# planck-epoch/unet-image-segmentation

Measured on AMD Instinct MI355X. Metric: images/sec (train step, 256x256x3), higher is better.
Workload: dtype f32; 1 GPU; configs[1]: 256x256x3 binary U-Net train step (fwd + dice_loss + bwd + AdamW + MeanIoU(2) update, dropout 0.2); network=U_NET separable-conv, filters 64-128-256-512, bneck 1024, global_batch=16, per_gpu_batch=16, seq_len=65536, parallelism=dp1, batchnorm=per-replica

## Files before the change

unet-image-segmentation_amd/csrc/gemm.hip:

```cpp
#include <cstdlib>
#include "dispatch.h"
#include "view.h"

namespace unet {

int colsum(const float* x, int64_t rows, int cols, float* out, void* ws, size_t ws_bytes, hipStream_t st);
size_t bn_partials_bytes(int64_t m, int c);
size_t colsum_workspace(int64_t rows, int cols);

namespace {

constexpr int BK = 16;

enum { A_PLAIN = 0, A_BNRELU = 1, A_UNSHUFFLE = 2, A_BNBWD = 3 };
enum { E_STORE = 0, E_STATS = 1, E_SHUFFLE = 2, E_BNPART = 3 };

struct RowsArgs {
    DView a;
    int64_t M;
    int K;
    int uH, uW, uf;
    const float* B;
    int64_t sbk, sbn;
    int N;
    float* C;
    int64_t ldc;
    const float* bias;
    float2* stats;
    int sH, sW, sf;
    const float* z;
    const float* coef;
    float* side;
    const float *bsc, *bsh, *bmu, *brs;
    float* bnpart;
    float ep_rate, ep_inv_keep;
    uint64_t ep_seed;
    int ko;
    const unsigned short* Bx;
};
#ifdef UNET_LAB_BUILD
#define ROWS_KO(g, bit) (((g).ko & (bit)) != 0)
#else
#define ROWS_KO(g, bit) false
#endif

__device__ __forceinline__ int acc_row(int r, int hi) { return (r & 3) + 8 * (r >> 2) + 4 * hi; }

__device__ __forceinline__ void xcd_group_order(int groups, int sibs, int& grp, int& sib) {
    grp = blockIdx.x;
    sib = blockIdx.y;
    if (sibs > 1 && (groups & 7) == 0) {
        const int L = blockIdx.x + blockIdx.y * groups, u = L >> 3;
        grp = (u / sibs) * 8 + (L & 7);
        sib = u % sibs;
    }
// ... 183 lines not shown
            if (hi == 0) red[wm * BN + col] = q;
        }
        __syncthreads();
        if (wm == 0 && hi == 0) {
#pragma unroll
            for (int tn = 0; tn < TN; ++tn) {
                const int col = wn * (BN / 2) + tn * 32 + lo;
                const int n = n0 + col;
                if (n < g.N) g.stats[(int64_t)blockIdx.x * g.N + n] = make_float2(mean[tn], red[col] + red[BN + col]);
            }
        }
    }
    if constexpr (EPI == E_SHUFFLE) {
        const int64_t hw = (int64_t)g.sH * g.sW;
#pragma unroll
        for (int tn = 0; tn < TN; ++tn) {
            const int n = n0 + wn * (BN / 2) + tn * 32 + lo;
            if (n >= g.N) continue;
            const int ab = n / g.sf;
            const int co = n - ab * g.sf;
            const int a = ab >> 1, b = ab & 1;
            const float bias = g.bias ? g.bias[co] : 0.f;
#pragma unroll
            for (int tm = 0; tm < TM; ++tm)
#pragma unroll
                for (int r = 0; r < 16; ++r) {
                    const int rr = wm * (BM / 2) + tm * 32 + acc_row(r, hi);
                    if (rr >= M_rem) continue;
                    const int64_t m = m0 + rr;
                    const int img = (int)(m / hw);
                    const int rem = (int)(m - img * hw);
                    const int i = rem / g.sW, j = rem - (rem / g.sW) * g.sW;
                    const int64_t o = ((int64_t)(img * 2 * g.sH + 2 * i + a) * (2 * g.sW) + 2 * j + b) * g.sf + co;
                    g.C[o] = acc[tm][tn][r] + bias;
                }
        }
    }
}

enum { W_PLAIN = 0, W_BNRELU = 1, W_UNSHUFFLE = 2, W_BNBWD = 3 };

struct WgradArgs {
    DView a;
    int P;
    int uH, uW, uf;
    DView b;
    int Q;
    int64_t M, mslice;
    float* slab;
    const float* bz;
    const float* bcoef;
    float* colpart;
    bool x6;
};

template <int BP, int BQ, int AMODE, bool ADROP, int BMODE, bool BDROP>
__global__ __launch_bounds__(256) void gemm_wgrad_kernel(WgradArgs g) {
    constexpr int LDA = BP + 4, LDB = BQ + 4;
    constexpr int TM = BP / 64, TN = BQ / 64;
    constexpr int AR = BP / 16, BR = BQ / 16;
    constexpr int AS = 256 / BP, BS = 256 / BQ;
    __shared__ float As[2][BK][LDA];
    __shared__ float Bs[2][BK][LDB];

    const int tid = threadIdx.x, lane = tid & 63, wave = tid >> 6;
    const int wp = wave >> 1, wq = wave & 1;
    const int lo = lane & 31, hi = lane >> 5;
    const int ntp = (g.P + BP - 1) / BP;
    const int p0 = (blockIdx.x % ntp) * BP;
    const int q0 = (blockIdx.x / ntp) * BQ;
    const int64_t mb = (int64_t)blockIdx.y * g.mslice;
    const int64_t me = mb + g.mslice < g.M ? mb + g.mslice : g.M;

    const int ap = tid % BP, amm = tid / BP;
    const int p = p0 + ap;
    const bool pv = p < g.P;
    float asc = 1.f, ash = 0.f;
    int poff = p;
    if constexpr (AMODE == W_BNRELU) {
        if (pv) {
            asc = g.a.sc0[p];
            ash = g.a.sh0[p];
        }
    }
    if constexpr (AMODE == W_UNSHUFFLE) {
        const int ab = p / g.uf;
        const int co = p - ab * g.uf;
        poff = (ab >> 1) * (2 * g.uW * g.uf) + (ab & 1) * g.uf + co;
    }
    const int bq = tid % BQ, bmm = tid / BQ;
    const int q = q0 + bq;
    const bool qv = q < g.Q;
    float bsc = 1.f, bsh = 0.f;
    if constexpr (BMODE == W_BNRELU) {
        if (qv) {
            bsc = g.b.sc0[q];
            bsh = g.b.sh0[q];
        }
    }

    float ra[AR], rb[BR];
    auto load_stage = [&](int64_t k0) {
#pragma unroll
        for (int r = 0; r < AR; ++r) {
            const int64_t m = k0 + amm + AS * r;
            float v = 0.f;
            if (pv && m < me) {
// ... 14 lines not shown
#pragma unroll
        for (int r = 0; r < BR; ++r) {
            const int64_t m = k0 + bmm + BS * r;
            float v = 0.f;
            if (qv && m < me) {
                v = g.b.src0[m * g.b.c0 + q];
                if constexpr (BMODE == W_BNRELU) v = bnrelu(v, bsc, bsh);
                if constexpr (BDROP) v *= drop_mult(g.b.seed, (uint64_t)m * g.b.C + q, g.b.rate, g.b.inv_keep);
            }
            rb[r] = v;
        }
    };
    auto store_stage = [&](int buf) {
#pragma unroll
        for (int r = 0; r < AR; ++r) As[buf][amm + AS * r][ap] = ra[r];
#pragma unroll
        for (int r = 0; r < BR; ++r) Bs[buf][bmm + BS * r][bq] = rb[r];
    };

    floatx16 acc[TM][TN];
#pragma unroll
    for (int tm = 0; tm < TM; ++tm)
#pragma unroll
        for (int tn = 0; tn < TN; ++tn)
#pragma unroll
            for (int r = 0; r < 16; ++r) acc[tm][tn][r] = 0.f;

    const int nk = (int)((me - mb + BK - 1) / BK);
    if (nk > 0) {
        load_stage(mb);
        store_stage(0);
    }
    __syncthreads();
    for (int kt = 0; kt < nk; ++kt) {
        const int buf = kt & 1;
        if (kt + 1 < nk) load_stage(mb + (int64_t)(kt + 1) * BK);
#pragma unroll
        for (int kk = 0; kk < BK / 2; ++kk) {
            float av[TM], bv[TN];
#pragma unroll
            for (int tm = 0; tm < TM; ++tm) av[tm] = As[buf][2 * kk + hi][wp * (BP / 2) + tm * 32 + lo];
#pragma unroll
            for (int tn = 0; tn < TN; ++tn) bv[tn] = Bs[buf][2 * kk + hi][wq * (BQ / 2) + tn * 32 + lo];
#pragma unroll
            for (int tm = 0; tm < TM; ++tm)
#pragma unroll
                for (int tn = 0; tn < TN; ++tn)
                    acc[tm][tn] = __builtin_amdgcn_mfma_f32_32x32x2f32(av[tm], bv[tn], acc[tm][tn], 0, 0, 0);
        }
        if (kt + 1 < nk) store_stage(buf ^ 1);
        __syncthreads();
    }
    float* slab = g.slab + (int64_t)blockIdx.y * g.P * g.Q;
#pragma unroll
    for (int tm = 0; tm < TM; ++tm)
#pragma unroll
        for (int tn = 0; tn < TN; ++tn) {
            const int qq = q0 + wq * (BQ / 2) + tn * 32 + lo;
            if (qq >= g.Q) continue;
#pragma unroll
            for (int r = 0; r < 16; ++r) {
                const int pp = p0 + wp * (BP / 2) + tm * 32 + acc_row(r, hi);
                if (pp < g.P) slab[(int64_t)pp * g.Q + qq] = acc[tm][tn][r];
            }
        }
}

#ifdef UNET_LAB_BUILD
__device__ __forceinline__ void lab_stagger(int ko) {
    const int n = (ko >> 8) & 255;
    if (n == 0) return;
    const unsigned lin = blockIdx.x + blockIdx.y * gridDim.x, tot = gridDim.x * gridDim.y;
    const bool late = (ko & 0x10000) ? (lin & 1) : (lin >= tot / 2);
    if (late)
        for (int i = 0; i < n; ++i) __builtin_amdgcn_s_sleep(32);
}
#define ROWS_STAGGER(g) lab_stagger((g).ko)
__device__ unsigned long long lab_rows_stamps[65536 * 4];
#define ROWS_STAMP(g, i)                                                                       \
    do {                                                                                       \
        if (((g).ko & 0x20000) && threadIdx.x == 0) {                                          \
            const unsigned lin_ = blockIdx.x + blockIdx.y * gridDim.x;                         \
            if (lin_ < 65536) lab_rows_stamps[4 * lin_ + (i)] =                               \
                ((i) == 0 || (i) == 3) ? __builtin_amdgcn_s_memrealtime() : __builtin_amdgcn_s_memtime(); \
        }                                                                                      \
    } while (0)
#else
#define ROWS_STAGGER(g) ((void)0)
#define ROWS_STAMP(g, i) ((void)0)
#endif

template <int BM, int BN, int BK, int AMODE, bool DROP, int EPI, bool BKC, bool X6 = false>
__global__ __launch_bounds__(256, X6 ? 2 : 1) void gemm_rows_vec(RowsArgs g) {
    main_stream_prio();
    ROWS_STAGGER(g);
    ROWS_STAMP(g, 0);
    constexpr int LR = BK + 4;
    constexpr int LB = BN + 4;
    constexpr int XR = BK + 8;
    constexpr int KQ = BK / 4;
    constexpr int NQ = BN / 4;
    constexpr int AQ = BM * KQ / 256;
    constexpr int BQ = BN * KQ / 256;
    constexpr int TM = BM / 64, TN = BN / 64;
    constexpr int BSZ = BKC ? BN * LR : BK * LB;
    constexpr int F32_BYTES = 4 * 2 * (BM * LR + BSZ);
    constexpr int X6_KMAX = 512;
    constexpr bool XCOEF = X6 && AMODE == A_BNBWD;
    constexpr int X6_BYTES = 2 * 3 * (BM + BN) * XR + (XCOEF ? 4 * 5 * X6_KMAX : 0);
    static_assert(!X6 || BK == 32, "X6 rows GEMM: 32-deep stages");
    __shared__ __attribute__((aligned(16))) char smem[X6 ? X6_BYTES : F32_BYTES];
    float* xcoef = reinterpret_cast<float*>(smem + 2 * 3 * (BM + BN) * XR);
    float (*As)[BM * LR] = reinterpret_cast<float (*)[BM * LR]>(smem);
    float (*Bs)[BSZ] = reinterpret_cast<float (*)[BSZ]>(smem + 4 * 2 * BM * LR);
    unsigned short* Ax = reinterpret_cast<unsigned short*>(smem);
    unsigned short* Bx = Ax + 3 * BM * XR;
    constexpr int XCH = BK / 8, XQ = 3 * BN * XCH / 256;
    static_assert(!X6 || (3 * BN * XCH) % 256 == 0, "X6: whole B chunks per thread");
// ... 348 lines not shown
                    }
                }
            }
            s1 += __shfl_xor(s1, 32, 64);
            s2 += __shfl_xor(s2, 32, 64);
            if (hi == 0) red[wm * BN + col] = make_float2(s1, s2);
        }
        __syncthreads();
        if (wm == 0 && hi == 0) {
            float* out = g.bnpart + (int64_t)mt * 2 * g.N;
#pragma unroll
            for (int tn = 0; tn < TN; ++tn) {
                const int col = wn * (BN / 2) + tn * 32 + lo;
                const int n = n0 + col;
                const float2 a = red[col], b = red[BN + col];
                if (n < g.N) {
                    out[n] = a.x + b.x;
                    out[g.N + n] = a.y + b.y;
                }
            }
        }
    }
    if constexpr (EPI == E_SHUFFLE) {
        int* orow = reinterpret_cast<int*>(&As[0][0]);
        if (tid < BM) {
            const int m = m0 + tid;
            const int ur = m / g.sW;
            orow[tid] = tid < M_rem ? (4 * ur * g.sW + 2 * (m - ur * g.sW)) * g.sf : -1;
        }
        __syncthreads();
        int obase[TM][16];
#pragma unroll
        for (int tm = 0; tm < TM; ++tm)
#pragma unroll
            for (int r = 0; r < 16; ++r) obase[tm][r] = orow[wm * (BM / 2) + tm * 32 + acc_row(r, hi)];
#pragma unroll
        for (int tn = 0; tn < TN; ++tn) {
            const int n = n0 + wn * (BN / 2) + tn * 32 + lo;
            if (n >= g.N) continue;
            const int ab = n / g.sf;
            const int co = n - ab * g.sf;
            const int toff = (ab >> 1) * (2 * g.sW * g.sf) + (ab & 1) * g.sf + co;
            const float bias = g.bias ? g.bias[co] : 0.f;
#pragma unroll
            for (int tm = 0; tm < TM; ++tm)
#pragma unroll
                for (int r = 0; r < 16; ++r)
                    if (obase[tm][r] >= 0) g.C[(int64_t)obase[tm][r] + toff] = acc[tm][tn][r] + bias;
        }
    }
    ROWS_STAMP(g, 3);
}

template <int BP, int BQ, int AMODE, bool ADROP, int BMODE, bool BDROP, bool X6 = false>
__global__ __launch_bounds__(256, X6 ? 2 : 1) void gemm_wgrad_vec(WgradArgs g) {
    static_assert(!X6 || (BP == 128 && BQ == 128), "X6 wgrad: 128 x 128 tiles");
    constexpr int KB = X6 ? 32 : BK;
    constexpr int LDA = BP + 4, LDB = BQ + 4;
    constexpr int TM = BP / 64, TN = BQ / 64;
    constexpr int PQ = BP / 4, QQ = BQ / 4;
    constexpr int AR = X6 ? 8 : BK * PQ / 256, BR = X6 ? 8 : BK * QQ / 256;
    constexpr int AS = X6 ? 1 : 256 / PQ, BS = X6 ? 1 : 256 / QQ;
    constexpr int XW = KB + 8;
    constexpr int F32_BYTES = 4 * 2 * BK * (LDA + LDB);
    constexpr int X6_BYTES = 2 * 3 * (BP + BQ) * XW;
    __shared__ __attribute__((aligned(16))) char smem[X6 ? X6_BYTES : F32_BYTES];
    float (*As)[BK * LDA] = reinterpret_cast<float (*)[BK * LDA]>(smem);
    float (*Bs)[BK * LDB] = reinterpret_cast<float (*)[BK * LDB]>(smem + 4 * 2 * BK * LDA);
    unsigned short* Ax = reinterpret_cast<unsigned short*>(smem);
    unsigned short* Bx = Ax + 3 * BP * XW;

    const int tid = threadIdx.x, lane = tid & 63, wave = tid >> 6;
    const int wp = wave >> 1, wq = wave & 1;
    const int lo = lane & 31, hi = lane >> 5;
    const int ntp = (g.P + BP - 1) / BP;
    int tile, slice;
    xcd_group_order_sx(gridDim.x, gridDim.y, tile, slice);
    const int p0 = (tile % ntp) * BP;
    const int q0 = (tile / ntp) * BQ;
    const int mb = (int)(slice * g.mslice);
    const int me = (int)((mb + g.mslice) < g.M ? (mb + g.mslice) : g.M);
    const bool roleA = !X6 || tid < 128, roleB = !X6 || tid >= 128;
    const int unit = tid & 127;

    const int apq = X6 ? unit >> 2 : tid % PQ, amm = X6 ? 8 * (unit & 3) : tid / PQ;
    const int p = p0 + 4 * apq;
    const bool pv = p < g.P;
    float4 asc = f4(1.f), ash = f4(0.f);
    int poff = p;
    if constexpr (AMODE == W_BNRELU) {
        if (pv) {
            asc = ld4(g.a.sc0 + p);
            ash = ld4(g.a.sh0 + p);
        }
    }
    if constexpr (AMODE == W_UNSHUFFLE) {
        const int ab = p / g.uf;
        const int co = p - ab * g.uf;
        poff = (ab >> 1) * (2 * g.uW * g.uf) + (ab & 1) * g.uf + co;
    }
    const int bqq = X6 ? unit >> 2 : tid % QQ, bmm = X6 ? 8 * (unit & 3) : tid / QQ;
    const int q = q0 + 4 * bqq;
    const bool qv = q < g.Q;
    float4 bsc = f4(1.f), bsh = f4(0.f), bmu = f4(0.f), bp_ = f4(0.f), bq_ = f4(0.f);
    if constexpr (BMODE == W_BNRELU || BMODE == W_BNBWD) {
        if (qv) {
            bsc = ld4(g.b.sc0 + q);
            bsh = ld4(g.b.sh0 + q);
// ... 24 lines not shown
            float4 v = f4(0.f);
            if (roleA && pv && m < me) {
                if constexpr (AMODE == W_UNSHUFFLE) {
                    v = ld4(g.a.src0 + (4 * ur[r] * g.uW + 2 * uj[r]) * g.uf + poff);
                } else {
                    v = ld4(g.a.src0 + (int64_t)m * g.a.c0 + p);
                    if constexpr (AMODE == W_BNRELU) v = bnrelu4(v, asc, ash);
                    if constexpr (ADROP) {
                        const uint64_t i = (uint64_t)m * g.a.C + p;
                        v = mul4(v, drop_mult4(g.a.seed, i, g.a.rate, g.a.inv_keep));
                    }
                }
            }
            ra[r] = v;
        }
#pragma unroll
        for (int r = 0; r < BR; ++r) {
            const int m = k0 + bmm + BS * r;
            float4 v = f4(0.f);
            if (roleB && qv && m < me) {
                v = ld4(g.b.src0 + (int64_t)m * g.b.c0 + q);
                if constexpr (BMODE == W_BNRELU) v = bnrelu4(v, bsc, bsh);
                if constexpr (BMODE == W_BNBWD) {
                    const float4 zz = ld4(g.bz + (int64_t)m * g.b.c0 + q);
                    v.x = fmaf(zz.x, bsc.x, bsh.x) > 0.f ? v.x : 0.f;
                    v.y = fmaf(zz.y, bsc.y, bsh.y) > 0.f ? v.y : 0.f;
                    v.z = fmaf(zz.z, bsc.z, bsh.z) > 0.f ? v.z : 0.f;
                    v.w = fmaf(zz.w, bsc.w, bsh.w) > 0.f ? v.w : 0.f;
                    v.x = bsc.x * (v.x - bp_.x - (zz.x - bmu.x) * bq_.x);
                    v.y = bsc.y * (v.y - bp_.y - (zz.y - bmu.y) * bq_.y);
                    v.z = bsc.z * (v.z - bp_.z - (zz.z - bmu.z) * bq_.z);
                    v.w = bsc.w * (v.w - bp_.w - (zz.w - bmu.w) * bq_.w);
                }
                if constexpr (BDROP) {
                    const uint64_t i = (uint64_t)m * g.b.C + q;
                    v = mul4(v, drop_mult4(g.b.seed, i, g.b.rate, g.b.inv_keep));
                }
            }
            rb[r] = v;
        }
        if constexpr (AMODE == W_UNSHUFFLE) {
#pragma unroll
            for (int r = 0; r < AR; ++r) {
                uj[r] += KB;
                while (uj[r] >= g.uW) {
                    uj[r] -= g.uW;
                    ++ur[r];
                }
            }
        }
    };
    const bool csum_on = g.colpart != nullptr && tile < ntp;
    float4 csum = f4(0.f);
    auto store_t4 = [&](unsigned short* base, int rows, const float4* rv) {
        const float4 cols[4] = {make_float4(rv[0].x, rv[1].x, rv[2].x, rv[3].x),
                                make_float4(rv[0].y, rv[1].y, rv[2].y, rv[3].y),
                                make_float4(rv[0].z, rv[1].z, rv[2].z, rv[3].z),
                                make_float4(rv[0].w, rv[1].w, rv[2].w, rv[3].w)};
#pragma unroll
        for (int c = 0; c < 4; ++c) {
            const Split4 sp = split4(cols[c]);
            unsigned short* d = base + c * XW;
            *reinterpret_cast<uint2*>(d) = sp.h;
            *reinterpret_cast<uint2*>(d + rows * XW) = sp.m;
            *reinterpret_cast<uint2*>(d + 2 * rows * XW) = sp.l;
        }
    };
    auto store_stage = [&](int buf) {
        if constexpr (X6) {
            if (roleA) {
                store_t4(Ax + 4 * apq * XW + amm, BP, ra);
                store_t4(Ax + 4 * apq * XW + amm + 4, BP, ra + 4);
            } else {
                store_t4(Bx + 4 * bqq * XW + bmm, BQ, rb);
                store_t4(Bx + 4 * bqq * XW + bmm + 4, BQ, rb + 4);
            }
        } else {
#pragma unroll
            for (int r = 0; r < AR; ++r) *reinterpret_cast<float4*>(&As[buf][(amm + AS * r) * LDA + 4 * apq]) = ra[r];
#pragma unroll
            for (int r = 0; r < BR; ++r) *reinterpret_cast<float4*>(&Bs[buf][(bmm + BS * r) * LDB + 4 * bqq]) = rb[r];
        }
        if (csum_on && roleA) {
#pragma unroll
            for (int r = 0; r < AR; ++r) csum = add4(csum, ra[r]);
        }
    };

    floatx16 acc[TM][TN];
#pragma unroll
    for (int tm = 0; tm < TM; ++tm)
#pragma unroll
        for (int tn = 0; tn < TN; ++tn)
#pragma unroll
            for (int r = 0; r < 16; ++r) acc[tm][tn][r] = 0.f;

    const int nk = (me - mb + KB - 1) / KB;
    if (nk > 0) {
        load_stage(mb);
        store_stage(0);
    }
    __syncthreads();
    for (int kt = 0; kt < nk; ++kt) {
        const int buf = kt & 1;
        if (kt + 1 < nk) load_stage(mb + (kt + 1) * KB);
        if constexpr (X6) {
#pragma unroll
            for (int ks = 0; ks < KB / 16; ++ks) {
                bf16x8 bfr[TN][3];
#pragma unroll
                for (int pl = 0; pl < 3; ++pl)
#pragma unroll
                    for (int tn = 0; tn < TN; ++tn)
                        bfr[tn][pl] = *reinterpret_cast<const bf16x8*>(
                            Bx + (pl * BQ + wq * (BQ / 2) + tn * 32 + lo) * XW + ks * 16 + 8 * hi);
#pragma unroll
                for (int tm = 0; tm < TM; ++tm) {
                    bf16x8 af[3];
#pragma unroll
                    for (int pl = 0; pl < 3; ++pl)
                        af[pl] = *reinterpret_cast<const bf16x8*>(
                            Ax + (pl * BP + wp * (BP / 2) + tm * 32 + lo) * XW + ks * 16 + 8 * hi);
#pragma unroll
                    for (int tn = 0; tn < TN; ++tn) acc[tm][tn] = mfma_x6(af, bfr[tn], acc[tm][tn]);
                }
            }
            __syncthreads();
            if (kt + 1 < nk) {
                store_stage(0);
                __syncthreads();
            }
            continue;
        } else {
#pragma unroll
        for (int kk = 0; kk < BK / 2; ++kk) {
            float av[TM], bv[TN];
#pragma unroll
            for (int tm = 0; tm < TM; ++tm) av[tm] = As[buf][(2 * kk + hi) * LDA + wp * (BP / 2) + tm * 32 + lo];
#pragma unroll
            for (int tn = 0; tn < TN; ++tn) bv[tn] = Bs[buf][(2 * kk + hi) * LDB + wq * (BQ / 2) + tn * 32 + lo];
#pragma unroll
            for (int tm = 0; tm < TM; ++tm)
#pragma unroll
                for (int tn = 0; tn < TN; ++tn)
                    acc[tm][tn] = __builtin_amdgcn_mfma_f32_32x32x2f32(av[tm], bv[tn], acc[tm][tn], 0, 0, 0);
        }
        }
        if (kt + 1 < nk) store_stage(buf ^ 1);
        __syncthreads();
    }
    if (csum_on) {
        float4* T = reinterpret_cast<float4*>(&As[0][0]);
        T[tid] = csum;
        __syncthreads();
        if constexpr (X6) {
            if (tid < PQ && p0 + 4 * tid < g.P) {
                float4 t = T[4 * tid];
                for (int j = 1; j < 4; ++j) t = add4(t, T[4 * tid + j]);
                st4(g.colpart + (int64_t)slice * g.P + p0 + 4 * tid, t);
            }
        } else if (tid < PQ && pv) {
            float4 t = T[tid];
            for (int j = 1; j < AS; ++j) t = add4(t, T[j * PQ + tid]);
            st4(g.colpart + (int64_t)slice * g.P + p, t);
        }
    }
    float* slab = g.slab + (int64_t)slice * g.P * g.Q;
#pragma unroll
    for (int tm = 0; tm < TM; ++tm)
#pragma unroll
        for (int tn = 0; tn < TN; ++tn) {
            const int qq = q0 + wq * (BQ / 2) + tn * 32 + lo;
            if (qq >= g.Q) continue;
#pragma unroll
            for (int r = 0; r < 16; ++r) {
                const int pp = p0 + wp * (BP / 2) + tm * 32 + acc_row(r, hi);
                if (pp < g.P) slab[(int64_t)pp * g.Q + qq] = acc[tm][tn][r];
            }
        }
}

template <int G, bool DWF = false>
__global__ __launch_bounds__(256) void img_pw_bwd_kernel(const float* __restrict__ da, const float* __restrict__ z,
                                                         int64_t M, const float* __restrict__ P,
                                                         const float* __restrict__ sc, const float* __restrict__ sh,
                                                         const float* __restrict__ coef, const float* __restrict__ y,
                                                         float* __restrict__ dy, float* __restrict__ wpart,
                                                         const float* __restrict__ x = nullptr, int H = 0, int W = 0) {
    main_stream_prio();
    constexpr int C = 4 * G, PPW = 64 / G, U = 4, PB = 4 * U * PPW;
    constexpr int NT = DWF ? (9 + G - 1) / G : 0;
    constexpr int SW = 4 * C + (DWF ? 36 : 0);
    __shared__ float4 red[4][4][G];
    __shared__ float4 rdk[4][DWF ? 9 : 1];
    float4 gacc[NT > 0 ? NT : 1];
#pragma unroll
    for (int i = 0; i < (NT > 0 ? NT : 1); ++i) gacc[i] = f4(0.f);
    const int lane = threadIdx.x & 63, wave = threadIdx.x >> 6;
    const int q = lane % G, ps = lane / G;
    const int c = 4 * q;
    const float4 csc = ld4(sc + c), csh = ld4(sh + c), cmu = ld4(coef + c), cp = ld4(coef + C + c),
                 cq = ld4(coef + 2 * C + c);
    float4 pk[4], wacc[4];
#pragma unroll
    for (int ci = 0; ci < 4; ++ci) {
        pk[ci] = ld4(P + ci * C + c);
        wacc[ci] = f4(0.f);
    }
    for (int64_t base = (int64_t)blockIdx.x * PB; base < M; base += (int64_t)gridDim.x * PB) {
        const int64_t p0 = base + wave * U * PPW + ps;
        float4 ra[U], rz[U], ry[U];
        float4 xn[U][NT > 0 ? NT : 1];
#pragma unroll
        for (int u = 0; u < U; ++u) {
            const int64_t m = p0 + u * PPW;
            const bool in = m < M;
            ra[u] = in ? ld4(da + m * C + c) : f4(0.f);
            rz[u] = in ? ld4(z + m * C + c) : f4(0.f);
            ry[u] = in ? ld4(y + m * 4) : f4(0.f);
            if constexpr (DWF) {
                const int mi = in ? (int)m : 0;
                const int hw = H * W;
                const int r = mi - (mi / hw) * hw, hh = r / W, ww = r - hh * W;
#pragma unroll
                for (int i = 0; i < NT; ++i) {
                    const int t = q + i * G, di = t / 3 - 1, dj = t % 3 - 1;
                    const bool ok = in && t < 9 && hh + di >= 0 && hh + di < H && ww + dj >= 0 && ww + dj < W;
                    xn[u][i] = ok ? ld4(x + (int64_t)(mi + di * W + dj) * 4) : f4(0.f);
                }
            }
        }
        float4 s[U];
// ... 177 lines not shown
                return 0;
            }
        }
        if constexpr (AMODE == A_UNSHUFFLE && EPI == E_BNPART) {
            if (convt_bnpart_bm(a.M, (int)a.N) == 64) {
                if (lab_knob("UNET_CONVT_BM64", 1) == 2) launch_rows_tile<128, 16, AMODE, DROP, EPI, false, 64>(a, st);
                else if (c.bk == 32) launch_rows_tile<64, 32, AMODE, DROP, EPI, false, 64>(a, st);
                else launch_rows_tile<64, 16, AMODE, DROP, EPI, false, 64>(a, st);
                UNET_CHECK_LAUNCH(what);
                return 0;
            }
        }
        with_int<6416, 6432, 12832, 25616, 12816>(100 * c.bn + c.bk, [&](auto T) {
            launch_rows_tile<T() / 100, T() % 100, AMODE, DROP, EPI>(a, st);
        });
        UNET_CHECK_LAUNCH(what);
        return 0;
    }
    if constexpr (AMODE == A_BNBWD || EPI == E_BNPART) {
        UNET_CHECK_ARG(false, "%s: needs channel counts divisible by 4 and 16-B aligned operands", what);
    } else {
        with_bucket<64, 128>((int)a.N, [&](auto BN) {
            dim3 grid((unsigned)cdiv(a.M, 128), (unsigned)cdiv(a.N, BN()));
            gemm_rows_kernel<128, BN(), AMODE, DROP, EPI><<<grid, 256, 0, st>>>(a);
        });
        UNET_CHECK_LAUNCH(what);
    }
    return 0;
}

struct WgradPlan {
    int bp, bq, tiles, S;
    int64_t mslice;
};
WgradPlan wgrad_plan(int64_t M, int P, int Q) {
    WgradPlan w;
    w.bp = P > 64 ? 128 : 64;
    w.bq = Q > 64 ? 128 : 64;
    w.tiles = (int)(cdiv(P, w.bp) * cdiv(Q, w.bq));
    int target = lab_knob("UNET_WGRAD_BLOCKS", 1024);
    if (target < 1) target = 1024;
    int64_t want = cdiv(target, w.tiles);
    int64_t maxs = M / lab_knob("UNET_WGRAD_MINROWS", 512);
    if (maxs < 1) maxs = 1;
    int64_t S = want < maxs ? want : maxs;
    if (S < 1) S = 1;
    w.mslice = cdiv(cdiv(M, S), BK) * BK;
    w.S = (int)cdiv(M, w.mslice);
    return w;
}

bool wgrad_x6() { return lab_knob("UNET_WGRAD_X6", 0) != 0; }

template <int AMODE, bool ADROP, int BMODE, bool BDROP>
void launch_wgrad_t(const WgradArgs& a, const WgradPlan& w, hipStream_t st) {
    dim3 grid((unsigned)w.tiles, (unsigned)w.S);
    const unsigned pad = (unsigned)lab_knob("UNET_WGRAD_LDSPAD", 0);
    const bool vec = a.P % 4 == 0 && a.Q % 4 == 0 && (AMODE != W_UNSHUFFLE || a.uf % 4 == 0) &&
                     (AMODE == W_UNSHUFFLE || a.a.c0 % 4 == 0) && a.b.c0 % 4 == 0 &&
                     ((uintptr_t)a.a.src0 | (uintptr_t)a.b.src0) % 16 == 0;
    const bool vk = vec || BMODE == W_BNBWD;
#ifdef UNET_LAB_BUILD
    if (vk && w.bp == 128 && w.bq == 128 && a.x6 && wgrad_x6()) {
        gemm_wgrad_vec<128, 128, AMODE, ADROP, BMODE, BDROP, true><<<grid, 256, pad, st>>>(a);
        return;
    }
#endif
    with_int<128, 64>(w.bp, [&](auto BP) {
        with_int<128, 64>(w.bq, [&](auto BQ) {
            if (vk) gemm_wgrad_vec<BP(), BQ(), AMODE, ADROP, BMODE, BDROP><<<grid, 256, pad, st>>>(a);
            else if constexpr (BMODE != W_BNBWD)
                gemm_wgrad_kernel<BP(), BQ(), AMODE, ADROP, BMODE, BDROP><<<grid, 256, pad, st>>>(a);
        });
    });
}

int run_wgrad(WgradArgs a, int amode, int bmode, float* out, void* ws, size_t ws_bytes, hipStream_t st,
              const char* what) {
    WgradPlan w = wgrad_plan(a.M, a.P, a.Q);
    const size_t need = (size_t)w.S * a.P * a.Q * sizeof(float);
    UNET_CHECK_ARG(ws && ws_bytes >= need, "%s: workspace %zu < %zu", what, ws_bytes, need);
    a.mslice = w.mslice;
    a.slab = static_cast<float*>(ws);
    a.x6 = true;
    const bool ad = a.a.rate > 0.f, bd = a.b.rate > 0.f;
    if (amode == W_PLAIN && bmode == W_PLAIN) {
        launch_wgrad_t<W_PLAIN, false, W_PLAIN, false>(a, w, st);
    } else if (amode == W_UNSHUFFLE && (bmode == W_BNRELU || bmode == W_PLAIN)) {
        with_int<W_BNRELU, W_PLAIN>(bmode, [&](auto BM) {
            with_bool(bd, [&](auto BD) { launch_wgrad_t<W_UNSHUFFLE, false, BM(), BD()>(a, w, st); });
        });
    } else if (amode == W_BNRELU && bmode == W_PLAIN) {
        with_bool(ad, [&](auto AD) { launch_wgrad_t<W_BNRELU, AD(), W_PLAIN, false>(a, w, st); });
    } else {
        UNET_CHECK_ARG(false, "%s: unsupported wgrad operand modes %d/%d", what, amode, bmode);
    }
    UNET_CHECK_LAUNCH(what);
    return reduce_slabs(a.slab, w.S, (int64_t)a.P * a.Q, out, (int64_t)a.P * a.Q, (int64_t)a.P * a.Q, st);
}

size_t wgrad_workspace(int64_t M, int P, int Q) {
    WgradPlan w = wgrad_plan(M, P, Q);
    return align_up((size_t)w.S * P * Q * sizeof(float), 256);
}

DView plain_view(const float* p, int c) {
    unet_view v{};
    v.mode = UNET_VIEW_PLAIN;
    v.c0 = c;
    v.src0 = p;
    return make_dview(v);
}

bool fits_i32(int64_t a, int64_t b) { return a * b < (int64_t(1) << 31); }

}
}

using namespace unet;

extern "C" size_t unet_bn_partials_size(int64_t m, int c) {
    if (m <= 0 || c <= 0) return 0;
    return bn_partials_bytes(m, c);
}

namespace {
int pw_fwd(const float* y, int64_t m, int cin, int cout, const float* pw_kernel, const unsigned short* pw_kernel_x3,
           float* z, float* bn_partials, unet_stream_t stream) {
    UNET_CHECK_ARG(y && pw_kernel && z, "unet_pointwise_fwd: null pointer");
    UNET_CHECK_ARG(m > 0 && cin > 0 && cout > 0, "unet_pointwise_fwd: bad sizes");
    UNET_CHECK_ARG(fits_i32(m, cin) && fits_i32(m, cout), "unet_pointwise_fwd: tensor too large");
    RowsArgs a{};
    a.a = plain_view(y, cin);
    a.M = m;
    a.K = cin;
    a.B = pw_kernel;
    a.Bx = pw_kernel_x3;
    a.sbk = cout;
    a.sbn = 1;
    a.N = cout;
    a.C = z;
    a.ldc = cout;
    a.stats = reinterpret_cast<float2*>(bn_partials);
    hipStream_t st = as_stream(stream);
    if (bn_partials) return launch_rows<A_PLAIN, false, E_STATS>(a, st, "unet_pointwise_fwd");
    return launch_rows<A_PLAIN, false, E_STORE>(a, st, "unet_pointwise_fwd");
}
}

extern "C" int unet_pointwise_fwd(const float* y, int64_t m, int cin, int cout, const float* pw_kernel, float* z,
// ... 298 lines not shown
    size_t a = wgrad_workspace(M, 4 * cout, cin) + align_up((size_t)wp.S * 4 * cout * sizeof(float), 256);
    size_t b = colsum_workspace(4 * M, cout);
    return a > b ? a : b;
}

extern "C" int unet_conv_transpose2x2_bwd(const unet_view* x, int n, int h, int w, int cout, const float* kernel,
                                          const float* dout, float* dx, float* dkernel, float* dbias, void* ws,
                                          size_t ws_bytes, unet_stream_t stream) {
    if (check_view(x, "unet_conv_transpose2x2_bwd")) return -1;
    UNET_CHECK_ARG(x->mode == UNET_VIEW_PLAIN || x->mode == UNET_VIEW_BNRELU,
                   "unet_conv_transpose2x2_bwd: input view must be PLAIN or BNRELU");
    UNET_CHECK_ARG(kernel && dout && n > 0 && h > 0 && w > 0 && cout > 0, "unet_conv_transpose2x2_bwd: bad args");
    UNET_CHECK_ARG((dkernel == nullptr) == (dbias == nullptr) && (dx || dkernel),
                   "unet_conv_transpose2x2_bwd: dkernel and dbias go together; nothing to compute");
    const int cin = x->c0;
    const int64_t M = (int64_t)n * h * w;
    UNET_CHECK_ARG(fits_i32(M, cin) && fits_i32(4 * M, cout), "unet_conv_transpose2x2_bwd: tensor too large");
    hipStream_t st = as_stream(stream);
    const size_t need = unet_conv_transpose2x2_bwd_workspace(n, h, w, cin, cout);
    UNET_CHECK_ARG(ws && ws_bytes >= need, "unet_conv_transpose2x2_bwd: workspace %zu < %zu", ws_bytes, need);
    if (dx) {
        RowsArgs a{};
        a.a = plain_view(dout, cout);
        a.M = M;
        a.K = 4 * cout;
        a.uH = h;
        a.uW = w;
        a.uf = cout;
        a.B = kernel;
        a.sbk = cin;
        a.sbn = 1;
        a.N = cin;
        a.C = dx;
        a.ldc = cin;
        int rc = launch_rows<A_UNSHUFFLE, false, E_STORE>(a, st, "unet_conv_transpose2x2_bwd(data)");
        if (rc) return rc;
    }
    if (!dkernel) return 0;
    WgradArgs wa{};
    wa.a = plain_view(dout, cout);
    wa.P = 4 * cout;
    wa.uH = h;
    wa.uW = w;
    wa.uf = cout;
    wa.b = make_dview(*x);
    wa.Q = cin;
    wa.M = M;
    const WgradPlan wp = wgrad_plan(M, 4 * cout, cin);
    const size_t slab_bytes = align_up((size_t)wp.S * 4 * cout * cin * sizeof(float), 256);
    const bool fuse_bias = convt_fused_bias() && cin % 4 == 0 && cout % 4 == 0 &&
                           ((uintptr_t)dout | (uintptr_t)x->src0) % 16 == 0 &&
                           ws_bytes >= slab_bytes + (size_t)wp.S * 4 * cout * sizeof(float);
    if (fuse_bias) wa.colpart = reinterpret_cast<float*>(static_cast<char*>(ws) + slab_bytes);
    int rc = run_wgrad(wa, W_UNSHUFFLE, x->mode == UNET_VIEW_BNRELU ? W_BNRELU : W_PLAIN, dkernel, ws, ws_bytes, st,
                       "unet_conv_transpose2x2_bwd(filter)");
    if (rc) return rc;
    if (fuse_bias) return reduce_slabs(wa.colpart, 4 * wp.S, cout, dbias, cout, cout, st);
    return colsum(dout, 4 * M, cout, dbias, ws, ws_bytes, st);
}

extern "C" int unet_conv_transpose2x2_bwd_data_bnstats_slabs(const unet_view* x, int n, int h, int w, int cout) {
    if (!x || x->mode != UNET_VIEW_BNRELU || !(x->drop_rate >= 0.f && x->drop_rate < 1.f) || n <= 0 || h <= 0 ||
        w <= 0 || cout <= 0)
        return 0;
    if (x->c0 % 4 || cout % 4) return 0;
    const int64_t M = (int64_t)n * h * w;
    if (!fits_i32(M, x->c0) || !fits_i32(4 * M, cout)) return 0;
    return (int)cdiv(M, convt_bnpart_bm(M, x->c0));
}

namespace {
int convt_bwd_data_bnstats(const unet_view* x, int n, int h, int w, int cout, const float* kernel,
                           const unsigned short* kernel_x3t, const float* dout, float* dx, const float* mean,
                           const float* rstd, float* bn_partials, unet_stream_t stream) {
    if (check_view(x, "unet_conv_transpose2x2_bwd_data_bnstats")) return -1;
    const int S = unet_conv_transpose2x2_bwd_data_bnstats_slabs(x, n, h, w, cout);
    UNET_CHECK_ARG(S > 0, "unet_conv_transpose2x2_bwd_data_bnstats: needs a BNRELU view (dropout rate in [0, 1)) "
                          "and channel counts divisible by 4");
    UNET_CHECK_ARG(kernel && dout && dx && bn_partials && x->scale0 && x->shift0,
                   "unet_conv_transpose2x2_bwd_data_bnstats: bad args");
    UNET_CHECK_ARG((mean == nullptr) == (rstd == nullptr), "unet_conv_transpose2x2_bwd_data_bnstats: mean/rstd go together");
    const int cin = x->c0;
    RowsArgs a{};
    a.a = plain_view(dout, cout);
    a.M = (int64_t)n * h * w;
    a.K = 4 * cout;
    a.uH = h;
    a.uW = w;
    a.uf = cout;
    a.B = kernel;
    a.Bx = convt_bnpart_bm(a.M, cin) == 128 ? kernel_x3t : nullptr;
    a.sbk = cin;
    a.sbn = 1;
    a.N = cin;
    a.C = dx;
    a.ldc = cin;
    a.z = x->src0;
    a.bsc = x->scale0;
    a.bsh = x->shift0;
    a.bmu = mean;
    a.brs = rstd;
    a.bnpart = bn_partials;
    a.ep_rate = x->drop_rate;
    a.ep_inv_keep = x->drop_rate > 0.f ? 1.0f / (1.0f - x->drop_rate) : 1.0f;
    a.ep_seed = x->drop_seed;
    UNET_CHECK_ARG(rows_vec_ok(a, A_UNSHUFFLE) && ((uintptr_t)dx | (uintptr_t)x->src0) % 16 == 0,
                   "unet_conv_transpose2x2_bwd_data_bnstats: operands must be 16-B aligned");
    return launch_rows<A_UNSHUFFLE, false, E_BNPART>(a, as_stream(stream), "unet_conv_transpose2x2_bwd_data_bnstats");
}
// ... 32 lines not shown
```

unet-image-segmentation_amd/csrc/lastblock.h:

```cpp
#pragma once
#include "common.h"

namespace unet {

constexpr int kGroupSlabs = 64;

inline size_t bnpart_scratch_off(int S, int C) { return align_up((size_t)S * 2 * C * sizeof(float), 256); }
inline size_t bnpart_counter_off(int S, int C) {
    return bnpart_scratch_off(S, C) + align_up((size_t)cdiv(S, kGroupSlabs) * 2 * C * sizeof(double), 256);
}
inline size_t bnpart_bytes(int S, int C) { return bnpart_counter_off(S, C) + (size_t)cdiv(C, 64) * sizeof(unsigned); }

__device__ __forceinline__ void st_agent(double* p, double v) {
    __hip_atomic_store(p, v, __ATOMIC_RELAXED, __HIP_MEMORY_SCOPE_AGENT);
}
template <typename T>
__device__ __forceinline__ T ld_agent(const T* p) {
    return __hip_atomic_load(p, __ATOMIC_RELAXED, __HIP_MEMORY_SCOPE_AGENT);
}

__device__ __forceinline__ bool last_arrival(unsigned* ctr, unsigned expected, int* flag) {
    asm volatile("s_waitcnt vmcnt(0)" ::: "memory");
    __syncthreads();
    if (threadIdx.x == 0) {
        const unsigned prev = __hip_atomic_fetch_add(ctr, 1u, __ATOMIC_RELAXED, __HIP_MEMORY_SCOPE_AGENT);
        const int last = prev == expected - 1;
        if (last) __hip_atomic_store(ctr, 0u, __ATOMIC_RELAXED, __HIP_MEMORY_SCOPE_AGENT);
        *flag = last;
    }
    __syncthreads();
    return *flag != 0;
}

}
```

Measured before the change: 1640 images/sec.

## Fuse split-K wgrad slab reduction into kernel via last-arriving block

Adds an in-kernel finish to the weight-gradient GEMMs. Each slice publishes its partial slab with agent-scope stores, and per-tile counters let the last-arriving block sum the slabs, plus the fused bias column partials, straight into the output. This is meant to remove the separate reduce_slabs and bias-reduction launches and their extra memory pass. It adds atomic counters, a cached per-stream counter buffer and serialized tail work in the last block. It is gated by a lab knob that defaults to off. Separately, the minimum blocks-per-CU launch bound for the vector wgrad kernel rises depending on tile shape, which constrains register allocation.

Result: no change. 1638 images/sec, median of 2 (-0.2%).

```diff
diff --git a/unet-image-segmentation_amd/csrc/gemm.hip b/unet-image-segmentation_amd/csrc/gemm.hip
--- a/unet-image-segmentation_amd/csrc/gemm.hip
+++ b/unet-image-segmentation_amd/csrc/gemm.hip
@@ -1,6 +1,11 @@
 #include <cstdlib>
+#include <mutex>
+#include <type_traits>
+#include <vector>
 #include "dispatch.h"
+#include "lastblock.h"
 #include "view.h"
+#include "wgrad_finish.h"
 
 namespace unet {
 
@@ -290,7 +295,95 @@
     const float* bcoef;
     float* colpart;
     bool x6;
+    unsigned* ctr;
+    float* out;
+    float* dbias;
 };
+
+template <int BP, int BQ, int W>
+__device__ __forceinline__ void wgrad_sum_slabs(const float* src, int64_t sp, int n, int P, int Q, int p0, int q0,
+                                                float* dst, bool publish) {
+    constexpr int QW = BQ / W, RP = 256 / QW;
+    const int q = q0 + W * ((int)threadIdx.x % QW);
+    if (q >= Q) return;
+    auto run = [&](auto UBT) {
+        constexpr int UB = decltype(UBT)::value;
+        for (int r = (int)threadIdx.x / QW; r < BP && p0 + r < P; r += RP) {
+            const int64_t o = (int64_t)(p0 + r) * Q + q;
+            double a[W];
+#pragma unroll
+            for (int k = 0; k < W; ++k) a[k] = 0.0;
+            for (int s = 0; s < n; s += UB) {
+                float v[UB][W];
+#pragma unroll
+                for (int u = 0; u < UB; ++u) {
+                    const float* x = src + (int64_t)(s + u < n ? s + u : n - 1) * sp + o;
+                    if constexpr (W == 4) {
+                        const float4 t = ld_agent4(x);
+                        v[u][0] = t.x; v[u][1] = t.y; v[u][2] = t.z; v[u][3] = t.w;
+                    } else {
+                        v[u][0] = ld_agent(x);
+                    }
+                }
+#pragma unroll
+                for (int u = 0; u < UB; ++u)
+                    if (s + u < n) {
+#pragma unroll
+                        for (int k = 0; k < W; ++k) a[k] += (double)v[u][k];
+                    }
+            }
+            if constexpr (W == 4) {
+                const float4 t = make_float4((float)a[0], (float)a[1], (float)a[2], (float)a[3]);
+                if (publish) st_agent(reinterpret_cast<float4*>(dst + o), t);
+                else {
+                    dst[o] = t.x; dst[o + 1] = t.y; dst[o + 2] = t.z; dst[o + 3] = t.w;
+                }
+            } else {
+                if (publish) st_agent(dst + o, (float)a[0]);
+                else dst[o] = (float)a[0];
+            }
+        }
+    };
+    constexpr int UMAX = W == 1 || (BP == 128 && BQ == 128) ? 16 : 8;
+    if (n <= 4) run(std::integral_constant<int, 4>{});
+    else if (n <= 8 || UMAX == 8) run(std::integral_constant<int, 8>{});
+    else run(std::integral_constant<int, UMAX>{});
+}
+
+template <int BP, int BQ, int W>
+__device__ __forceinline__ void wgrad_finish(const WgradArgs& g, int tile, int slice, int p0, int q0, bool csum_on,
+                                             int* flag) {
+    const int tiles = gridDim.x, S = gridDim.y;
+    const int NG = finish_groups(S), grp = slice / kFinishGroup;
+    const int64_t sp = (int64_t)g.P * g.Q;
+    if (!last_arrival(g.ctr + finish_group_counter(tiles, S, tile, grp), (unsigned)finish_group_size(S, grp), flag))
+        return;
+    const int s0 = grp * kFinishGroup, gs = finish_group_size(S, grp);
+    if (NG == 1) {
+        wgrad_sum_slabs<BP, BQ, W>(g.slab, sp, gs, g.P, g.Q, p0, q0, g.out, false);
+        if (csum_on) wgrad_sum_slabs<1, BP, 4>(g.colpart, g.P, gs, 1, g.P, 0, p0, g.colpart, true);
+    } else {
+        float* lead = g.slab + (int64_t)s0 * sp;
+        wgrad_sum_slabs<BP, BQ, W>(lead, sp, gs, g.P, g.Q, p0, q0, lead, true);
+        if (csum_on) wgrad_sum_slabs<1, BP, 4>(g.colpart + (int64_t)s0 * g.P, g.P, gs, 1, g.P, 0, p0,
+                                               g.colpart + (int64_t)s0 * g.P, true);
+        if (!last_arrival(g.ctr + finish_tile_counter(tiles, S, tile), (unsigned)NG, flag)) return;
+        wgrad_sum_slabs<BP, BQ, W>(g.slab, kFinishGroup * sp, NG, g.P, g.Q, p0, q0, g.out, false);
+        if (csum_on) wgrad_sum_slabs<1, BP, 4>(g.colpart, (int64_t)kFinishGroup * g.P, NG, 1, g.P, 0, p0, g.colpart, true);
+    }
+    if (!csum_on) return;
+    const int ntp = (g.P + BP - 1) / BP;
+    if (!last_arrival(g.ctr + finish_bias_counter(tiles, S), (unsigned)ntp, flag)) return;
+    for (int co = threadIdx.x; co < g.uf; co += 256) {
+        float v[4];
+#pragma unroll
+        for (int ab = 0; ab < 4; ++ab) v[ab] = ld_agent(g.colpart + ab * g.uf + co);
+        double t = 0.0;
+#pragma unroll
+        for (int ab = 0; ab < 4; ++ab) t += (double)v[ab];
+        g.dbias[co] = (float)t;
+    }
+}
 
 template <int BP, int BQ, int AMODE, bool ADROP, int BMODE, bool BDROP>
 __global__ __launch_bounds__(256) void gemm_wgrad_kernel(WgradArgs g) {
@@ -411,6 +504,7 @@
         __syncthreads();
     }
     float* slab = g.slab + (int64_t)blockIdx.y * g.P * g.Q;
+    const bool fin = g.ctr != nullptr;
 #pragma unroll
     for (int tm = 0; tm < TM; ++tm)
 #pragma unroll
@@ -420,9 +514,13 @@
 #pragma unroll
             for (int r = 0; r < 16; ++r) {
                 const int pp = p0 + wp * (BP / 2) + tm * 32 + acc_row(r, hi);
-                if (pp < g.P) slab[(int64_t)pp * g.Q + qq] = acc[tm][tn][r];
-            }
-        }
+                if (pp < g.P) {
+                    if (fin) st_agent(slab + (int64_t)pp * g.Q + qq, acc[tm][tn][r]);
+                    else slab[(int64_t)pp * g.Q + qq] = acc[tm][tn][r];
+                }
+            }
+        }
+    if (fin) wgrad_finish<BP, BQ, 1>(g, (int)blockIdx.x, (int)blockIdx.y, p0, q0, false, reinterpret_cast<int*>(&As[0][0][0]));
 }
 
 #ifdef UNET_LAB_BUILD
@@ -877,8 +975,15 @@
     ROWS_STAMP(g, 3);
 }
 
+template <int BP, int BQ, int AMODE, bool ADROP, int BMODE, bool BDROP>
+constexpr int wgrad_vec_waves() {
+    if (BP + BQ == 256) return 4;
+    if (BP + BQ == 192) return 5;
+    return AMODE == W_UNSHUFFLE && BMODE == W_BNRELU && BDROP ? 6 : 7;
+}
 template <int BP, int BQ, int AMODE, bool ADROP, int BMODE, bool BDROP, bool X6 = false>
-__global__ __launch_bounds__(256, X6 ? 2 : 1) void gemm_wgrad_vec(WgradArgs g) {
+__global__ __launch_bounds__(256, (X6 ? 2 : wgrad_vec_waves<BP, BQ, AMODE, ADROP, BMODE, BDROP>()))
+void gemm_wgrad_vec(WgradArgs g) {
     static_assert(!X6 || (BP == 128 && BQ == 128), "X6 wgrad: 128 x 128 tiles");
     constexpr int KB = X6 ? 32 : BK;
     constexpr int LDA = BP + 4, LDB = BQ + 4;
@@ -1009,6 +1114,7 @@
     };
     const bool csum_on = g.colpart != nullptr && tile < ntp;
     float4 csum = f4(0.f);
+    const bool fin = g.ctr != nullptr;
     auto store_t4 = [&](unsigned short* base, int rows, const float4* rv) {
         const float4 cols[4] = {make_float4(rv[0].x, rv[1].x, rv[2].x, rv[3].x),
                                 make_float4(rv[0].y, rv[1].y, rv[2].y, rv[3].y),
@@ -1114,12 +1220,16 @@
             if (tid < PQ && p0 + 4 * tid < g.P) {
                 float4 t = T[4 * tid];
                 for (int j = 1; j < 4; ++j) t = add4(t, T[4 * tid + j]);
-                st4(g.colpart + (int64_t)slice * g.P + p0 + 4 * tid, t);
+                float* cp = g.colpart + (int64_t)slice * g.P + p0 + 4 * tid;
+                if (fin) st_agent(reinterpret_cast<float4*>(cp), t);
+                else st4(cp, t);
             }
         } else if (tid < PQ && pv) {
             float4 t = T[tid];
             for (int j = 1; j < AS; ++j) t = add4(t, T[j * PQ + tid]);
-            st4(g.colpart + (int64_t)slice * g.P + p, t);
+            float* cp = g.colpart + (int64_t)slice * g.P + p;
+            if (fin) st_agent(reinterpret_cast<float4*>(cp), t);
+            else st4(cp, t);
         }
     }
     float* slab = g.slab + (int64_t)slice * g.P * g.Q;
@@ -1132,9 +1242,13 @@
 #pragma unroll
             for (int r = 0; r < 16; ++r) {
                 const int pp = p0 + wp * (BP / 2) + tm * 32 + acc_row(r, hi);
-                if (pp < g.P) slab[(int64_t)pp * g.Q + qq] = acc[tm][tn][r];
-            }
-        }
+                if (pp < g.P) {
+                    if (fin) st_agent(slab + (int64_t)pp * g.Q + qq, acc[tm][tn][r]);
+                    else slab[(int64_t)pp * g.Q + qq] = acc[tm][tn][r];
+                }
+            }
+        }
+    if (fin) wgrad_finish<BP, BQ, 4>(g, tile, slice, p0, q0, csum_on, reinterpret_cast<int*>(smem));
 }
 
 template <int G, bool DWF = false>
@@ -1418,13 +1532,48 @@
 
 bool wgrad_x6() { return lab_knob("UNET_WGRAD_X6", 0) != 0; }
 
+bool wgrad_vec_ok(const WgradArgs& a, int amode) {
+    return a.P % 4 == 0 && a.Q % 4 == 0 && (amode != W_UNSHUFFLE || a.uf % 4 == 0) &&
+           (amode == W_UNSHUFFLE || a.a.c0 % 4 == 0) && a.b.c0 % 4 == 0 &&
+           ((uintptr_t)a.a.src0 | (uintptr_t)a.b.src0) % 16 == 0;
+}
+
+unsigned* wgrad_finish_counters(hipStream_t st) {
+    struct Entry {
+        int dev;
+        hipStream_t st;
+        unsigned* ctr;
+    };
+    static std::mutex mu;
+    static std::vector<Entry> table;
+    int dev = 0;
+    if (hipGetDevice(&dev) != hipSuccess) return nullptr;
+    std::lock_guard<std::mutex> lock(mu);
+    for (const Entry& e : table)
+        if (e.dev == dev && e.st == st) return e.ctr;
+    hipStreamCaptureStatus cap = hipStreamCaptureStatusNone;
+    if (hipStreamIsCapturing(st, &cap) != hipSuccess || cap != hipStreamCaptureStatusNone) {
+        (void)hipGetLastError();
+        return nullptr;
+    }
+    unsigned* p = nullptr;
+    if (hipMalloc(&p, kFinishCounters * sizeof(unsigned)) != hipSuccess ||
+        hipMemsetAsync(p, 0, kFinishCounters * sizeof(unsigned), st) != hipSuccess) {
+        (void)hipGetLastError();
+        if (p) (void)hipFree(p);
+        return nullptr;
+    }
+    table.push_back({dev, st, p});
+    return p;
+}
+
+bool wgrad_finish_on() { return lab_knob("UNET_WGRAD_FINISH", 0) != 0; }
+
 template <int AMODE, bool ADROP, int BMODE, bool BDROP>
 void launch_wgrad_t(const WgradArgs& a, const WgradPlan& w, hipStream_t st) {
     dim3 grid((unsigned)w.tiles, (unsigned)w.S);
     const unsigned pad = (unsigned)lab_knob("UNET_WGRAD_LDSPAD", 0);
-    const bool vec = a.P % 4 == 0 && a.Q % 4 == 0 && (AMODE != W_UNSHUFFLE || a.uf % 4 == 0) &&
-                     (AMODE == W_UNSHUFFLE || a.a.c0 % 4 == 0) && a.b.c0 % 4 == 0 &&
-                     ((uintptr_t)a.a.src0 | (uintptr_t)a.b.src0) % 16 == 0;
+    const bool vec = wgrad_vec_ok(a, AMODE);
     const bool vk = vec || BMODE == W_BNBWD;
 #ifdef UNET_LAB_BUILD
     if (vk && w.bp == 128 && w.bq == 128 && a.x6 && wgrad_x6()) {
@@ -1442,13 +1591,23 @@
 }
 
 int run_wgrad(WgradArgs a, int amode, int bmode, float* out, void* ws, size_t ws_bytes, hipStream_t st,
-              const char* what) {
+              const char* what, float* dbias = nullptr, bool* bias_done = nullptr) {
     WgradPlan w = wgrad_plan(a.M, a.P, a.Q);
     const size_t need = (size_t)w.S * a.P * a.Q * sizeof(float);
     UNET_CHECK_ARG(ws && ws_bytes >= need, "%s: workspace %zu < %zu", what, ws_bytes, need);
     a.mslice = w.mslice;
     a.slab = static_cast<float*>(ws);
     a.x6 = true;
+    const bool vec = wgrad_vec_ok(a, amode);
+    const bool fin_ok = vec ? ((uintptr_t)a.slab | (uintptr_t)a.colpart) % 16 == 0 && (!a.colpart || dbias)
+                            : a.colpart == nullptr;
+    const long long fin_max = (long long)lab_knob("UNET_WGRAD_FINISH_MAXKB", (int)(kFinishMaxBytes >> 10)) << 10;
+    const bool fin_pays = fin_max == 0 || finish_block_bytes(a.P, a.Q, w.bp, w.bq, w.S) <= fin_max;
+    if (wgrad_finish_on() && fin_ok && fin_pays && finish_counter_count(w.tiles, w.S) > 0)
+        a.ctr = wgrad_finish_counters(st);
+    a.out = out;
+    a.dbias = dbias;
+    if (bias_done) *bias_done = a.ctr != nullptr && a.colpart != nullptr;
     const bool ad = a.a.rate > 0.f, bd = a.b.rate > 0.f;
     if (amode == W_PLAIN && bmode == W_PLAIN) {
         launch_wgrad_t<W_PLAIN, false, W_PLAIN, false>(a, w, st);
@@ -1462,6 +1621,7 @@
         UNET_CHECK_ARG(false, "%s: unsupported wgrad operand modes %d/%d", what, amode, bmode);
     }
     UNET_CHECK_LAUNCH(what);
+    if (a.ctr) return 0;
     return reduce_slabs(a.slab, w.S, (int64_t)a.P * a.Q, out, (int64_t)a.P * a.Q, (int64_t)a.P * a.Q, st);
 }
 
@@ -1866,9 +2026,11 @@
                            ((uintptr_t)dout | (uintptr_t)x->src0) % 16 == 0 &&
                            ws_bytes >= slab_bytes + (size_t)wp.S * 4 * cout * sizeof(float);
     if (fuse_bias) wa.colpart = reinterpret_cast<float*>(static_cast<char*>(ws) + slab_bytes);
+    bool bias_done = false;
     int rc = run_wgrad(wa, W_UNSHUFFLE, x->mode == UNET_VIEW_BNRELU ? W_BNRELU : W_PLAIN, dkernel, ws, ws_bytes, st,
-                       "unet_conv_transpose2x2_bwd(filter)");
+                       "unet_conv_transpose2x2_bwd(filter)", fuse_bias ? dbias : nullptr, &bias_done);
     if (rc) return rc;
+    if (bias_done) return 0;
     if (fuse_bias) return reduce_slabs(wa.colpart, 4 * wp.S, cout, dbias, cout, cout, st);
     return colsum(dout, 4 * M, cout, dbias, ws, ws_bytes, st);
 }
diff --git a/unet-image-segmentation_amd/csrc/lastblock.h b/unet-image-segmentation_amd/csrc/lastblock.h
--- a/unet-image-segmentation_amd/csrc/lastblock.h
+++ b/unet-image-segmentation_amd/csrc/lastblock.h
@@ -14,9 +14,25 @@
 __device__ __forceinline__ void st_agent(double* p, double v) {
     __hip_atomic_store(p, v, __ATOMIC_RELAXED, __HIP_MEMORY_SCOPE_AGENT);
 }
+__device__ __forceinline__ void st_agent(float* p, float v) {
+    __hip_atomic_store(p, v, __ATOMIC_RELAXED, __HIP_MEMORY_SCOPE_AGENT);
+}
 template <typename T>
 __device__ __forceinline__ T ld_agent(const T* p) {
     return __hip_atomic_load(p, __ATOMIC_RELAXED, __HIP_MEMORY_SCOPE_AGENT);
+}
+__device__ __forceinline__ void st_agent(float4* p, float4 v) {
+    unsigned long long* q = reinterpret_cast<unsigned long long*>(p);
+    const unsigned long long lo = (unsigned long long)__float_as_uint(v.x) | ((unsigned long long)__float_as_uint(v.y) << 32);
+    const unsigned long long hi = (unsigned long long)__float_as_uint(v.z) | ((unsigned long long)__float_as_uint(v.w) << 32);
+    __hip_atomic_store(q, lo, __ATOMIC_RELAXED, __HIP_MEMORY_SCOPE_AGENT);
+    __hip_atomic_store(q + 1, hi, __ATOMIC_RELAXED, __HIP_MEMORY_SCOPE_AGENT);
+}
+__device__ __forceinline__ float4 ld_agent4(const float* p) {
+    const unsigned long long* q = reinterpret_cast<const unsigned long long*>(p);
+    const unsigned long long lo = ld_agent(q), hi = ld_agent(q + 1);
+    return make_float4(__uint_as_float((unsigned)lo), __uint_as_float((unsigned)(lo >> 32)),
+                       __uint_as_float((unsigned)hi), __uint_as_float((unsigned)(hi >> 32)));
 }
 
 __device__ __forceinline__ bool last_arrival(unsigned* ctr, unsigned expected, int* flag) {
diff --git a/unet-image-segmentation_amd/csrc/wgrad_finish.h b/unet-image-segmentation_amd/csrc/wgrad_finish.h
--- /dev/null
+++ b/unet-image-segmentation_amd/csrc/wgrad_finish.h
@@ -0,0 +1,34 @@
+#pragma once
+
+#if defined(__HIPCC__) || defined(__CUDACC__)
+#define UNET_HD __host__ __device__
+#else
+#define UNET_HD
+#endif
+
+namespace unet {
+
+constexpr int kFinishGroup = 32;
+constexpr int kFinishCounters = 8192;
+
+constexpr long long kFinishMaxBytes = 128 << 10;
+UNET_HD inline long long finish_block_bytes(int P, int Q, int bp, int bq, int S) {
+    const int gs = S < kFinishGroup ? S : kFinishGroup;
+    return (long long)(P < bp ? P : bp) * (Q < bq ? Q : bq) * 4 * gs;
+}
+
+UNET_HD inline int finish_groups(int S) { return (S + kFinishGroup - 1) / kFinishGroup; }
+UNET_HD inline int finish_group_size(int S, int grp) {
+    const int left = S - grp * kFinishGroup;
+    return left < kFinishGroup ? left : kFinishGroup;
+}
+UNET_HD inline int finish_group_counter(int tiles, int S, int tile, int grp) { return tile * finish_groups(S) + grp; }
+UNET_HD inline int finish_tile_counter(int tiles, int S, int tile) { return tiles * finish_groups(S) + tile; }
+UNET_HD inline int finish_bias_counter(int tiles, int S) { return tiles * finish_groups(S) + tiles; }
+UNET_HD inline int finish_counter_count(int tiles, int S) {
+    if (tiles < 1 || S < 1) return 0;
+    const long long n = (long long)tiles * finish_groups(S) + tiles + 1;
+    return n <= kFinishCounters ? (int)n : 0;
+}
+
+}
```
